# openxrlab/xrsfm

Measured on AMD Instinct MI355X. Metric: BA iterations/sec x (cams+points), higher is better.
Workload: dtype f64; 1 GPU; synthetic BAL-style L: 1000 cams / 500000 points / 2000000 obs, GBA accurate (ba_solver.cc:626-629), seed 4; parallelism=single GPU, linear_solver=cholesky (explicit reduced camera matrix, exact)

## Files before the change

### include/xrsfm_ba.h

```cpp
#ifndef XRSFM_BA_H
#define XRSFM_BA_H

#include <stddef.h>
#include <stdint.h>

#ifdef __cplusplus
extern "C" {
#endif

#define XRSFM_BA_VERSION 1

#define XRSFM_BA_OK 0
#define XRSFM_BA_EINVAL (-1)
#define XRSFM_BA_ENODEV (-2)
#define XRSFM_BA_ENOMEM (-3)
#define XRSFM_BA_ECOMM (-4)
#define XRSFM_BA_ESTATE (-5)
#define XRSFM_BA_ETOOBIG (-6)
#define XRSFM_BA_EINTERNAL (-7)
#define XRSFM_BA_ESINGULAR (-8)

#define XRSFM_BA_SIMPLE_PINHOLE 0
#define XRSFM_BA_PINHOLE 1
#define XRSFM_BA_SIMPLE_RADIAL 2
// ... 302 lines not shown

int xrsfm_ba_debug_gram_schedule(int n_cams, int32_t *n_inst, int32_t *n_inst_all, uint16_t *entries);

int xrsfm_ba_debug_chol_plan(const xrsfm_ba_problem *problem, int32_t stats[8], int32_t *cam_offset, int32_t *facts);

int xrsfm_ba_debug_device_pack_check(const xrsfm_ba_problem *problem, int32_t *field, int32_t *index);

int xrsfm_ba_debug_set_block_pattern(xrsfm_ba_context *ctx, int n_pairs, const int32_t *row_col);

int xrsfm_ba_debug_cholesky_solve(xrsfm_ba_context *ctx, double radius, double *y, double *S_dense);

int xrsfm_ba_debug_reduced_system(xrsfm_ba_context *ctx, double radius, int32_t facts[16], int32_t *n_blocks, int32_t *blk_rc,
                                  double *blk, double *diag, double *b, double *y);

int xrsfm_ba_debug_wide(xrsfm_ba_context *ctx, double huber_a, double radius, double *cost, double *r, double *Jc, double *Jp,
                        double *Hcc_diag, double *gc, double *y);

int xrsfm_ba_debug_backsub(xrsfm_ba_context *ctx, double *part_model, double *part_step2, double *cand_points,
                           double *point_step, double *cand_cam_q, double *cand_cam_t);

int xrsfm_ba_debug_backsub_layout(xrsfm_ba_context *ctx, int32_t *pt_orig, int32_t *item_tiles, double *campart, int32_t flags[2],
                                  double *cand_intr, double *scale_c, double *scale_p);

int xrsfm_ba_debug_stored_j(xrsfm_ba_context *ctx, int32_t *stored);

int xrsfm_ba_debug_lin_scalars(xrsfm_ba_context *ctx, double out[4]);

#ifdef __cplusplus
}
#endif
#endif
```

### xrsfm_amd/capi.py

```python
from __future__ import annotations

import ctypes as C
import os

import numpy as np

from . import _build

_c_double_p = C.POINTER(C.c_double)
_c_int32_p = C.POINTER(C.c_int32)
_c_uint8_p = C.POINTER(C.c_uint8)


class CProblem(C.Structure):
    _fields_ = [
        ("n_cams", C.c_int32), ("n_points", C.c_int32), ("n_obs", C.c_int32), ("n_intr", C.c_int32),
        ("cam_q", _c_double_p), ("cam_t", _c_double_p), ("cam_const", _c_uint8_p), ("cam_intr", _c_int32_p),
        ("intr_model", _c_int32_p), ("intr_params", _c_double_p),
        ("points", _c_double_p), ("point_const", _c_uint8_p),
        ("obs_cam", _c_int32_p), ("obs_pt", _c_int32_p), ("obs_uv", _c_double_p),
    ]


class CPgProblem(C.Structure):
# ... 71 lines not shown
        ("total_time_s", C.c_double), ("dom_kernel_ms", C.c_double),
        ("dom_kernel_launches", C.c_int32), ("dom_kernel_id", C.c_int32),
        ("linear_solver_used", C.c_int32), ("reserved", C.c_int32),
    ]

    def as_dict(self):
        return {f: getattr(self, f) for f, _ in self._fields_}


EXPORTS = [
    "xrsfm_ba_default_options", "xrsfm_ba_version", "xrsfm_ba_create", "xrsfm_ba_comm_unique_id",
    "xrsfm_ba_comm_init", "xrsfm_ba_run", "xrsfm_ba_reset", "xrsfm_ba_download", "xrsfm_ba_destroy",
    "xrsfm_ba_solve", "xrsfm_ba_filter_tracks", "xrsfm_ba_profile_entry", "xrsfm_ba_debug_linearize", "xrsfm_ba_debug_schur_product",
    "xrsfm_ba_debug_cholesky_solve", "xrsfm_ba_debug_set_block_pattern", "xrsfm_ba_debug_pack", "xrsfm_ba_debug_chol_plan", "xrsfm_ba_refine_pose", "xrsfm_ba_refine_pose_options", "xrsfm_ba_debug_comm_hook", "xrsfm_pg_default_options", "xrsfm_pg_solve", "xrsfm_ba_debug_pack_gram", "xrsfm_ba_debug_gram_schedule",
    "xrsfm_tag_default_options", "xrsfm_tag_refine", "xrsfm_ba_refine_poses", "xrsfm_ba_quiesce", "xrsfm_ba_debug_backsub", "xrsfm_ba_device_memory", "xrsfm_ba_download_intrinsics", "xrsfm_ba_debug_wide",
    "xrsfm_ba_debug_device_pack_check", "xrsfm_ba_warmup", "xrsfm_ba_debug_stored_j", "xrsfm_ba_debug_sgroup",
    "xrsfm_ba_debug_reduced_system", "xrsfm_ba_covariance", "xrsfm_ba_point_covariance", "xrsfm_ba_joint_covariance",
    "xrsfm_ba_map_covariance", "xrsfm_ba_debug_backsub_layout", "xrsfm_ba_run_batch", "xrsfm_ba_solve_batch",
    "xrsfm_ba_triangulate_options", "xrsfm_ba_triangulate_tracks", "xrsfm_ba_debug_lin_scalars",
    "xrsfm_ba_absolute_pose_options", "xrsfm_ba_absolute_pose", "xrsfm_ba_debug_pose_samples",
    "xrsfm_ba_two_view_options_default", "xrsfm_ba_two_view_init", "xrsfm_ba_debug_two_view_samples",
    "xrsfm_ba_verify_pairs_options", "xrsfm_ba_verify_pairs", "xrsfm_ba_debug_fund_samples",
    "xrsfm_ba_match_options_default", "xrsfm_ba_match_descriptors", "xrsfm_ba_debug_match_table",
]
EXPORTS_WITH_DIGITS = ["xrsfm_ba_debug_match_top2"]

CHOL_FACTS = ("T", "levels", "ordering", "schedule", "macro_levels", "split_levels", "la_depth", "fill_rest", "rest_apart", "packed",
              "bwd", "height_mask", "cw", "blocks", "n", "tiles_nz")
SCHEDULES = ("level", "panel", "lookahead")
BWD_FORMS = ("fused", "per_level", "all", "chunk", "push")


def _facts(v) -> dict:
    f = dict(zip(CHOL_FACTS, (int(x) for x in v)))
    f["schedule"] = SCHEDULES[f["schedule"]]
    f["bwd"] = BWD_FORMS[f["bwd"]]
    f["rest_apart"] = bool(f["rest_apart"]); f["packed"] = bool(f["packed"])
    f["heights"] = sorted(m * f["cw"] for m in range(1, 31) if (f["height_mask"] >> m) & 1)
    return f

SOLVER_PCG, SOLVER_CHOLESKY, SOLVER_AUTO = 0, 1, 2
SOLVER_RESIDENT = 3
BATCH_MAX = 4096
TRI_MAX_OBS = 128
TRI_LOCAL_BIT = 1 << 30
POSE_MAX_CORR = 8192
# ... 36 lines not shown
    lib.xrsfm_ba_run.argtypes = [vp, C.POINTER(COptions), C.POINTER(CSummary)]; lib.xrsfm_ba_run.restype = C.c_int
    lib.xrsfm_ba_reset.argtypes = [vp]; lib.xrsfm_ba_reset.restype = C.c_int
    lib.xrsfm_ba_download.argtypes = [vp, _c_double_p, _c_double_p, _c_double_p]; lib.xrsfm_ba_download.restype = C.c_int
    lib.xrsfm_ba_destroy.argtypes = [vp]; lib.xrsfm_ba_destroy.restype = None
    lib.xrsfm_ba_solve.argtypes = [C.POINTER(COptions), C.POINTER(CProblem), C.POINTER(CSummary)]; lib.xrsfm_ba_solve.restype = C.c_int
    lib.xrsfm_ba_filter_tracks.argtypes = [C.POINTER(CProblem), C.c_double, C.c_double, _c_uint8_p, _c_uint8_p, _c_double_p,
                                            _c_double_p, _c_int32_p]
    lib.xrsfm_ba_filter_tracks.restype = C.c_int
    lib.xrsfm_ba_debug_linearize.argtypes = [vp, C.c_double, C.c_int] + [_c_double_p] * 8
    lib.xrsfm_ba_debug_linearize.restype = C.c_int
    lib.xrsfm_ba_debug_schur_product.argtypes = [vp, C.c_double, _c_double_p, _c_double_p, _c_double_p]
    lib.xrsfm_ba_debug_schur_product.restype = C.c_int
    lib.xrsfm_ba_debug_cholesky_solve.argtypes = [vp, C.c_double, _c_double_p, _c_double_p]
    lib.xrsfm_ba_debug_cholesky_solve.restype = C.c_int
    if hasattr(lib, "xrsfm_ba_debug_stored_j"):
        lib.xrsfm_ba_debug_stored_j.argtypes = [vp, C.POINTER(C.c_int32)]
        lib.xrsfm_ba_debug_stored_j.restype = C.c_int
    if hasattr(lib, "xrsfm_ba_debug_backsub"):
        lib.xrsfm_ba_debug_backsub.argtypes = [vp] + [_c_double_p] * 6
        lib.xrsfm_ba_debug_backsub.restype = C.c_int
    if hasattr(lib, "xrsfm_ba_debug_backsub_layout"):
        lib.xrsfm_ba_debug_backsub_layout.argtypes = [vp, _c_int32_p, _c_int32_p, _c_double_p, _c_int32_p] + [_c_double_p] * 3
        lib.xrsfm_ba_debug_backsub_layout.restype = C.c_int
    lib.xrsfm_ba_debug_set_block_pattern.argtypes = [vp, C.c_int, _c_int32_p]
    lib.xrsfm_ba_debug_set_block_pattern.restype = C.c_int
    lib.xrsfm_pg_default_options.argtypes = [C.POINTER(CPgOptions)]
    lib.xrsfm_pg_default_options.restype = None
    lib.xrsfm_ba_refine_poses.argtypes = [C.POINTER(COptions), C.c_int32, _c_int32_p, _c_double_p, _c_int32_p, _c_double_p, _c_double_p,
                                          _c_uint8_p, _c_double_p, _c_double_p, C.POINTER(CSummary)]
    lib.xrsfm_ba_refine_poses.restype = C.c_int
    lib.xrsfm_pg_solve.argtypes = [C.POINTER(CPgOptions), C.POINTER(CPgProblem), C.POINTER(CPgSummary)]
    lib.xrsfm_pg_solve.restype = C.c_int
    lib.xrsfm_tag_default_options.argtypes = [C.POINTER(CPgOptions)]
    lib.xrsfm_tag_default_options.restype = None
    lib.xrsfm_tag_refine.argtypes = [C.POINTER(CPgOptions), C.POINTER(CTagProblem), C.c_int32, C.POINTER(CPgSummary)]
    lib.xrsfm_tag_refine.restype = C.c_int
    lib.xrsfm_ba_debug_comm_hook.argtypes = [C.c_void_p, C.c_int, C.c_int, ALLREDUCE_FN, C.c_void_p]
    lib.xrsfm_ba_debug_comm_hook.restype = C.c_int
    lib.xrsfm_ba_refine_pose_options.argtypes = [C.POINTER(COptions)]
    lib.xrsfm_ba_refine_pose_options.restype = None
    lib.xrsfm_ba_refine_pose.argtypes = [C.POINTER(COptions), C.c_int32, _c_double_p, C.c_int32, _c_double_p, _c_double_p, _c_uint8_p,
                                         _c_double_p, _c_double_p, C.POINTER(CSummary)]
    lib.xrsfm_ba_refine_pose.restype = C.c_int
    lib.xrsfm_ba_debug_pack_gram.argtypes = [C.POINTER(CProblem), _c_int32_p, _c_int32_p, _c_uint8_p, _c_int32_p]
    lib.xrsfm_ba_debug_pack_gram.restype = C.c_int
    lib.xrsfm_ba_debug_sgroup.argtypes = [C.POINTER(CProblem), C.c_int] + [_c_int32_p] * 7
# ... 304 lines not shown
        p = self.problem
        out = dict(r=np.zeros((p.n_obs, 2)), Jc=np.zeros((p.n_obs, 2, 9)), Jp=np.zeros((p.n_obs, 2, 3)), Hcc_diag=np.zeros((p.n_cams, 9)),
                   gc=np.zeros((p.n_cams, 9)))
        y = np.zeros((p.n_cams, 9)) if radius is not None else None
        cost = C.c_double(0)
        self.lib.xrsfm_ba_debug_wide.argtypes = [C.c_void_p, C.c_double, C.c_double, C.POINTER(C.c_double)] + [_c_double_p] * 6
        self.lib.xrsfm_ba_debug_wide.restype = C.c_int
        check(self.lib.xrsfm_ba_debug_wide(self._h, huber_a, float(radius or 1.0), C.byref(cost), _dp(out["r"]), _dp(out["Jc"]), _dp(out["Jp"]),
                                          _dp(out["Hcc_diag"]), _dp(out["gc"]), _dp(y)), "xrsfm_ba_debug_wide")
        out["cost"] = cost.value
        if y is not None:
            out["y"] = y
        return out

    def debug_backsub(self) -> dict:
        st = debug_pack(self.problem)
        ni, npk, nc = st["items"], st["active_points"], self.problem.n_cams
        out = dict(part_model=np.zeros(ni), part_step2=np.zeros(ni), cand_points=np.zeros((npk, 3)), point_step=np.zeros((npk, 3)),
                   cand_cam_q=np.zeros((nc, 4)), cand_cam_t=np.zeros((nc, 3)))
        check(self.lib.xrsfm_ba_debug_backsub(self._h, *[_dp(out[k]) for k in ("part_model", "part_step2", "cand_points", "point_step",
                                                                                  "cand_cam_q", "cand_cam_t")]), "debug_backsub")
        return out

    def debug_backsub_layout(self, after_backsub: bool = False, scales: bool = False) -> dict:
        st = debug_pack(self.problem)
        nc = self.problem.n_cams
        out = dict(pt_orig=np.zeros(st["active_points"], np.int32), item_tiles=np.zeros((st["items"], 2), np.int32))
        flags = np.zeros(2, np.int32)
        if after_backsub:
            out["campart"] = np.zeros((2, nc)); out["cand_intr"] = np.zeros((nc, 3))
        if scales:
            cw = 9 if (self.problem.cam_const & 4).any() else 6
            out["scale_c"] = np.zeros((nc, cw)); out["scale_p"] = np.zeros((st["active_points"], 3))
        i32 = lambda a: a.ctypes.data_as(_c_int32_p)
        check(self.lib.xrsfm_ba_debug_backsub_layout(self._h, i32(out["pt_orig"]), i32(out["item_tiles"]), _dp(out.get("campart")), i32(flags),
                                                     _dp(out.get("cand_intr")), _dp(out.get("scale_c")), _dp(out.get("scale_p"))),
              "debug_backsub_layout")
        out["step_prep"] = bool(flags[0]); out["stored_j"] = bool(flags[1])
        out["slot_obs"] = st["slot_obs"]
        return out

    def debug_backsub_caller_order(self) -> dict:
        raw = self.debug_backsub()
        lay = self.debug_backsub_layout(after_backsub=True, scales=True)
        p = self.problem
        po = lay["pt_orig"]
# ... 552 lines not shown
```

### xrsfm_amd/csrc/ba_chol.h

```cpp
#pragma once
#include "ba_kernels.h"
#include "ba_pack.h"

namespace xba {

constexpr int kNB = 64;
constexpr int kLdT = 66;
constexpr int kCamsPerTileDev = 10;

struct CholDev {
    int n, n_pad, T;
    double* S;
    const int* tmap; size_t ld; size_t tstride;
    double* Linv;
    double* y;
    double* rhs;
    double* x;
    const int* cam_off;
    const int* tile_rows;
    int cw, cpt;
};

__device__ __forceinline__ double* tile_ptr(const CholDev& c, int i, int k) {
    return c.tmap ? c.S + (size_t)c.tmap[i * c.T + k] * c.tstride : c.S + (size_t)(i * kNB) * c.ld + k * kNB;
// ... 294 lines not shown
    double* const smem = smem_all + (size_t)wave * wld;
    XBA_STAMP(0, 0);
    SGroup sg{0, 1, smem, wld, 0.0, 0.0, -1};
    if (MERGED && sgrp) {
        const int code = __builtin_amdgcn_readfirstlane(sgrp[pos]);
        sg.idx = code & 15; sg.len = code >> 4;
    }
    const int entry = item_list[MERGED ? n_list - 1 - pos : pos];
    Item it;
    if (GRAM) { it.first_tile = entry; it.n_tiles = 1; }
    else it = d.items[entry];
    if (GRAM || it.n_tiles == 1) {
        int dt0 = -1, dt1 = -1;
        int g4_se = 0, g4_n = 0;
        if (GRAM) {
            const int C0 = d.tile_ncam[it.first_tile];
            const int* src = pair_dst + n_obs_pairs + d.tile_gt_off[it.first_tile];
            const int a0 = lane / kGramTabLd, b0 = lane - kGramTabLd * a0;
            const int a1 = (lane + kWave) / kGramTabLd, b1 = lane + kWave - kGramTabLd * a1;
            if (b0 > a0 && b0 < C0) dt0 = src[a0 * C0 + b0];
            if (b1 > a1 && b1 < C0 && a1 < kGramTabLd) dt1 = src[a1 * C0 + b1];
            if (NIK <= 2 && gram4) g4_se = gram4_sched_load<6>(C0, lane, g4_n);
        }
        const SlotCtx s = load_slot(d, it.first_tile, lane);
        const int cp = d.slot_campos_s[s.slot];
        const int cidx_raw = GRAM ? (int)d.slot_cidx[s.slot] : 0;
        const int L = d.tile_stride[it.first_tile];
        int g_pos = kWave - 1, g_pk0 = 0, g_pk1 = 0, g_pk2 = 0;
        if (GRAM && L == 0) {
            const int C0 = d.tile_ncam[it.first_tile];
            const int* trun = d.tile_run + (size_t)it.first_tile * kTileRunLd;
            const int c0 = lane / 14, c1 = (lane + 64) / 14, c2 = (lane + 128) / 14;
            g_pos = (int)d.slot_gpos[s.slot];
            if (c0 < C0) g_pk0 = trun[c0];
            if (c1 < C0) g_pk1 = trun[c1];
            if (c2 < C0) g_pk2 = trun[c2];
        }
        double V[18];
        int npair = 0, pbase = 0;
        {
            double o28[28];
            XBA_STAMP(0, 1);
            if (s.valid) {
                double hcv[6], gv[3];
                {
                    const double* hc = (PREP ? d.Hpp : d.Hc) + 6 * (size_t)s.pt;
                    const double* g = d.gp + 3 * (size_t)s.pt;
#pragma unroll
                    for (int k = 0; k < 6; ++k) hcv[k] = hc[k];
                    gv[0] = g[0]; gv[1] = g[1]; gv[2] = g[2];
                }
                double F[12], E[6], r0, r1;
                load_FE_rc(d, s.slot, s.cam, s.pt, F, E, r0, r1);
                if (PREP) { double hf[6]; point_factor(hcv, radius, hf);
#pragma unroll
                    for (int k = 0; k < 6; ++k) hcv[k] = hf[k]; }
                XBA_STAMP(0, 2);
                pairs_V<PREP>(F, E, hcv, V);
                XBA_STAMP(0, 3);
                pairs_diag<PREP>(F, V, hcv, gv, o28);
            } else if (PREP) { dead_values(V); dead_values(o28); }
            else {
#pragma unroll
                for (int k = 0; k < 18; ++k) V[k] = XBA_DEAD;
#pragma unroll
                for (int k = 0; k < 28; ++k) o28[k] = XBA_DEAD;
// ... 1407 lines not shown
```

### xrsfm_amd/csrc/ba_kernels.h

```cpp
#pragma once
#include "ba_math.h"

namespace xba {

constexpr int kWave = 64;
constexpr int kBlock = 256;
constexpr int kWavesPerBlock = kBlock / kWave;

struct Item { int first_tile; int n_tiles; };

struct PcgStatus {
    double rz;
    double rr;
    double bb;
    double pq;
    int it;
    int done;
    unsigned arrived;
};

enum Scal {
    S_COST = 0, S_XNORM2_PTS, S_MODEL, S_STEP2_PTS, S_COST_CAND, S_STEP2_CAMS, S_XNORM2_CAMS,
    S_GRADMAX_PTS, S_GRADMAX_CAMS,
    S_BWD_ERR,
    S_COUNT = 16
};

struct __attribute__((aligned(16))) CamLin {
    double M[9];
    double sq[3];
    double st[3];
    double pad;
};
static_assert(sizeof(CamLin) == 128, "CamLin must be 128 bytes");

struct Dev {
    int n_cams, n_pts, n_tiles, n_slots, n_items;
    const int* slot_cam; const int* slot_pt; const int* slot_campos;
    const double* slot_u; const double* slot_v;
    const Item* items;
    const int* tile_stride;
    const int* tile_maxlen;
    const int* tile_ncam;
    const int* tile_gt_off;
    const unsigned char* slot_cidx;
    const int* slot_campos_g;
    const unsigned char* slot_gpos;
    const int* tile_run;
    const int* cam_ptr_g;
    const int* slot_campos_s; const int* cam_ptr_s;
    CamRec* cam; CamRec* cam_cand; const int* cam_model; const unsigned char* cam_const; const int* cam_ptr;
    double* cam_act;
    double* P; double* P_cand; const unsigned char* pt_const;
    double* scale_c; double* scale_p;
    double* rt; double* Jp;
    double huber_a;
    CamLin* camrec;
    double* Hpp; double* gp; double* Hinv;
    double* Hc;
    double* camlin;
// ... 178 lines not shown
__global__ __launch_bounds__(256) void k_sgroup_remap_ptr(const int* __restrict__ src, int n, const int* __restrict__ pos, int* __restrict__ dst) {
    const int i = blockIdx.x * 256 + threadIdx.x;
    if (i < n) dst[i] = pos[src[i]];
}

struct SlotCtx {
    int slot, cam, pt, lane;
    bool valid, head;
};

__device__ __forceinline__ SlotCtx load_slot(const Dev& d, int tile, int lane) {
    SlotCtx s;
    s.lane = lane;
    s.slot = tile * kWave + lane;
    s.cam = d.slot_cam[s.slot];
    s.pt = d.slot_pt[s.slot];
    s.valid = s.cam >= 0;
    const int prev = __shfl_up(s.pt, 1, kWave);
    s.head = s.valid && (lane == 0 || prev != s.pt);
    return s;
}


__device__ __forceinline__ void robust_obs(const double (&M)[9], const double t[3], const double* intr, int model, const double Pw[3],
                                           double u, double v, double huber_a, Proj& pr, double& rho, double& sw) {
    project<true>(M, t, intr, model, Pw, u, v, pr);
    double rho1;
    rho = huber(pr.r0 * pr.r0 + pr.r1 * pr.r1, huber_a, rho1);
    sw = sqrt(rho1);
}

__device__ __forceinline__ void obs_rj(const Dev& d, int slot, int cam, const double (&M)[9], const double Pw[3],
                                       double& r0, double& r1, double (&j)[6]) {
    const CamRec& c = d.cam[cam];
    const double t[3] = {c.t[0], c.t[1], c.t[2]};
    Proj pr;
    double rho, sw;
    robust_obs(M, t, c.intr, d.cam_model[cam], Pw, d.slot_u[slot], d.slot_v[slot], d.huber_a, pr, rho, sw);
    r0 = pr.r0 * sw; r1 = pr.r1 * sw;
#pragma unroll
    for (int k = 0; k < 6; ++k) j[k] = pr.jp[k] * sw;
    asm("" : "+v"(r0), "+v"(r1));
#pragma unroll
    for (int k = 0; k < 6; ++k) asm("" : "+v"(j[k]));
}

__device__ __forceinline__ void fe_from_j(const Dev& d, const CamLin& c, const double (&M)[9], int pt, const double P0, const double P1,
                                          const double P2, const double (&j)[6], double (&F)[12], double (&E)[6]) {
    const double rp0 = M[0] * P0 + M[1] * P1 + M[2] * P2;
    const double rp1 = M[3] * P0 + M[4] * P1 + M[5] * P2;
    const double rp2 = M[6] * P0 + M[7] * P1 + M[8] * P2;
    const double* spp = d.scale_p + 3 * (size_t)pt;
    const double mp = d.pt_const[pt] ? 0.0 : 1.0;
    const double sp0 = spp[0] * mp, sp1 = spp[1] * mp, sp2 = spp[2] * mp;
#pragma unroll
    for (int row = 0; row < 2; ++row) {
        const double a = j[3 * row], b = j[3 * row + 1], cc = j[3 * row + 2];
        F[6 * row + 0] = -2.0 * (b * rp2 - cc * rp1) * c.sq[0];
        F[6 * row + 1] = -2.0 * (cc * rp0 - a * rp2) * c.sq[1];
        F[6 * row + 2] = -2.0 * (a * rp1 - b * rp0) * c.sq[2];
        F[6 * row + 3] = a * c.st[0];
        F[6 * row + 4] = b * c.st[1];
        F[6 * row + 5] = cc * c.st[2];
        E[3 * row + 0] = (a * M[0] + b * M[3] + cc * M[6]) * sp0;
        E[3 * row + 1] = (a * M[1] + b * M[4] + cc * M[7]) * sp1;
        E[3 * row + 2] = (a * M[2] + b * M[5] + cc * M[8]) * sp2;
    }
}

__device__ __forceinline__ void load_FE(const Dev& d, int slot, int cam, int pt, double (&F)[12], double (&E)[6]) {
    const size_t ns = (size_t)d.n_slots;
    double j[6];
#pragma unroll
    for (int k = 0; k < 6; ++k) j[k] = d.Jp[k * ns + slot];
    const CamLin& c = d.camrec[cam];
    double M[9];
#pragma unroll
    for (int k = 0; k < 9; ++k) M[k] = c.M[k];
    const double* P = d.P + 3 * (size_t)pt;
    fe_from_j(d, c, M, pt, P[0], P[1], P[2], j, F, E);
}

__device__ __forceinline__ void load_FE_rc(const Dev& d, int slot, int cam, int pt, double (&F)[12], double (&E)[6], double& r0, double& r1) {
    const size_t ns = (size_t)d.n_slots;
    const CamLin& c = d.camrec[cam];
    double M[9];
#pragma unroll
    for (int k = 0; k < 9; ++k) M[k] = c.M[k];
    const double* P = d.P + 3 * (size_t)pt;
    const double Pw[3] = {P[0], P[1], P[2]};
    double j[6];
    if (d.Jp) {
#pragma unroll
        for (int k = 0; k < 6; ++k) j[k] = d.Jp[k * ns + slot];
        r0 = d.rt[slot]; r1 = d.rt[ns + slot];
    } else {
        obs_rj(d, slot, cam, M, Pw, r0, r1, j);
    }
    fe_from_j(d, c, M, pt, Pw[0], Pw[1], Pw[2], j, F, E);
}

__device__ __forceinline__ void cam_lin_one(const Dev& d, int c, const double q[4], CamLin* __restrict__ out) {
    CamLin r;
    quat_to_mat(q, r.M);
    const unsigned cc = d.cam_const[c];
    const double* sc = d.scale_c + 6 * (size_t)c;
    for (int k = 0; k < 3; ++k) { r.sq[k] = (cc & 1u) ? 0.0 : sc[k]; r.st[k] = (cc & 2u) ? 0.0 : sc[3 + k]; }
    r.pad = 0.0;
    out[c] = r;
}
__global__ void k_cam_lin(Dev d) {
    const int c = blockIdx.x * blockDim.x + threadIdx.x;
    if (c >= d.n_cams) return;
    const double q[4] = {d.cam[c].q[0], d.cam[c].q[1], d.cam[c].q[2], d.cam[c].q[3]};
    cam_lin_one(d, c, q, d.camrec);
}

template <bool LONG>
__device__ __forceinline__ void linearize_item(const Dev& d, const Item& it, int item, int lane, double huber_a) {
    constexpr bool is_long = LONG;
    extern __shared__ __attribute__((aligned(16))) double lin_smem_acc[];
    double* acc = lin_smem_acc + (threadIdx.x >> 6) * (kWave * 13);
// ... 1120 lines not shown
            const int slot = (it.first_tile + tl) * kWave + lane;
            const int cam = d.slot_cam[slot];
            if (cam >= 0) {
                const double* y = d.px + 6 * (size_t)cam;
                double F[12], E[6], r0, r1;
                load_FE_rc(d, slot, cam, pt0, F, E, r0, r1);
                double v0 = 0.0, v1 = 0.0;
#pragma unroll
                for (int k = 0; k < 6; ++k) { v0 += F[k] * y[k]; v1 += F[6 + k] * y[k]; }
                const double m0 = v0 + E[0] * u[0] + E[1] * u[1] + E[2] * u[2];
                const double m1 = v1 + E[3] * u[0] + E[4] * u[1] + E[5] * u[2];
                model += m0 * (r0 - 0.5 * m0) + m1 * (r1 - 0.5 * m1);
            }
        }
    }
}

#if XBA_BACKSUB_WAVES > 0
#define XBA_BACKSUB_LEAN_WAVES XBA_BACKSUB_WAVES
#else
#define XBA_BACKSUB_LEAN_WAVES 5
#endif
constexpr int kBsLdsH = 16 * kWave, kBsLdsW = 4 * kWave;
constexpr int kBsLdsWave = 4 * kBsLdsH + 2 * kBsLdsW;

__device__ __forceinline__ double rounded(double x) { asm("" : "+v"(x)); return x; }

__device__ __forceinline__ void load_vE_rc(const Dev& d, int slot, int cam, const double (&Pw)[3], const double* __restrict__ sp, double mp,
                                           double (&spm)[3], double (&E)[6], double& v0, double& v1, double& r0, double& r1) {
    const size_t ns = (size_t)d.n_slots;
    const CamLin& c = d.camrec[cam];
    double M[9];
#pragma unroll
    for (int k = 0; k < 9; ++k) M[k] = c.M[k];
    double j[6];
    if (d.Jp) {
#pragma unroll
        for (int k = 0; k < 6; ++k) j[k] = d.Jp[k * ns + slot];
        r0 = d.rt[slot]; r1 = d.rt[ns + slot];
    } else {
        obs_rj(d, slot, cam, M, Pw, r0, r1, j);
    }
    const double rp0 = M[0] * Pw[0] + M[1] * Pw[1] + M[2] * Pw[2];
    const double rp1 = M[3] * Pw[0] + M[4] * Pw[1] + M[5] * Pw[2];
    const double rp2 = M[6] * Pw[0] + M[7] * Pw[1] + M[8] * Pw[2];
    const double* y = d.px + 6 * (size_t)cam;
#pragma unroll
    for (int k = 0; k < 3; ++k) spm[k] = sp[k] * mp;
    double v[2];
#pragma unroll
    for (int row = 0; row < 2; ++row) {
        const double a = j[3 * row], b = j[3 * row + 1], cc = j[3 * row + 2];
        double vr = 0.0;
        vr += -2.0 * (b * rp2 - cc * rp1) * c.sq[0] * y[0];
        vr += -2.0 * (cc * rp0 - a * rp2) * c.sq[1] * y[1];
        vr += -2.0 * (a * rp1 - b * rp0) * c.sq[2] * y[2];
        vr += a * c.st[0] * y[3];
        vr += b * c.st[1] * y[4];
        vr += cc * c.st[2] * y[5];
        v[row] = vr;
        E[3 * row + 0] = (a * M[0] + b * M[3] + cc * M[6]) * spm[0];
        E[3 * row + 1] = (a * M[1] + b * M[4] + cc * M[7]) * spm[1];
        E[3 * row + 2] = (a * M[2] + b * M[5] + cc * M[8]) * spm[2];
    }
    v0 = v[0]; v1 = v[1];
}

template <bool PREP, bool YP>
__global__ __launch_bounds__(kBlock) __attribute__((amdgpu_waves_per_eu(XBA_BACKSUB_LEAN_WAVES, XBA_BACKSUB_LEAN_WAVES)))
void k_backsub(Dev d, int n_item_blocks, CamLin* __restrict__ camrec_cand, double radius) {
    typedef __attribute__((address_space(1))) const void* gptr;
    typedef __attribute__((address_space(3))) void* lptr;
    __shared__ __attribute__((aligned(16))) unsigned char hg[kWavesPerBlock * kBsLdsWave];
    if ((int)blockIdx.x >= n_item_blocks) {
        const int c = (blockIdx.x - n_item_blocks) * kBlock + threadIdx.x;
        if (c < d.n_cams) cam_update_one(d, c, d.px + 6 * (size_t)c, camrec_cand);
        return;
    }
    const int lane = threadIdx.x & (kWave - 1);
    const int wave = __builtin_amdgcn_readfirstlane(threadIdx.x >> 6);
    const int item = blockIdx.x * kWavesPerBlock + wave;
    if (item >= d.n_items) return;
    const Item it = d.items[item];
    if (it.n_tiles != 1) return;
    const SlotCtx s = load_slot(d, it.first_tile, lane);
    const int maxlen = d.tile_maxlen[it.first_tile];
    unsigned char* const lw = hg + wave * kBsLdsWave;
    if (s.head) {
        const double* h = (PREP ? d.Hpp : d.Hinv) + 6 * (size_t)s.pt;
        const unsigned char* g = reinterpret_cast<const unsigned char*>(d.gp + 3 * (size_t)s.pt);
        __builtin_amdgcn_global_load_lds((gptr)h, (lptr)lw, 16, 0, 0);
        __builtin_amdgcn_global_load_lds((gptr)(h + 2), (lptr)(lw + kBsLdsH), 16, 0, 0);
        __builtin_amdgcn_global_load_lds((gptr)(h + 4), (lptr)(lw + 2 * kBsLdsH), 16, 0, 0);
        __builtin_amdgcn_global_load_lds((gptr)g, (lptr)(lw + 3 * kBsLdsH), 16, 0, 0);
        __builtin_amdgcn_global_load_lds((gptr)(g + 16), (lptr)(lw + 4 * kBsLdsH), 4, 0, 0);
        __builtin_amdgcn_global_load_lds((gptr)(g + 20), (lptr)(lw + 4 * kBsLdsH + kBsLdsW), 4, 0, 0);
    }
    double model = 0.0, step2 = 0.0;
    double E[6], v0, v1, r0, r1;
    double w[3] = {0, 0, 0};
    double spm[3], Pv[3];
    bool var = false;
    if (s.valid) {
        const double* P = d.P + 3 * (size_t)s.pt;
        var = !d.pt_const[s.pt];
        const double mp = var ? 1.0 : 0.0;
#pragma unroll
        for (int k = 0; k < 3; ++k) Pv[k] = P[k];
        load_vE_rc(d, s.slot, s.cam, Pv, d.scale_p + 3 * (size_t)s.pt, mp, spm, E, v0, v1, r0, r1);
#pragma unroll
        for (int k = 0; k < 3; ++k) w[k] = rounded(E[k] * v0) + E[3 + k] * v1;
    } else { dead_values(spm); dead_values(Pv); dead_values(E); XBA_DEAD_VALUE(v0); XBA_DEAD_VALUE(v1); XBA_DEAD_VALUE(r0); XBA_DEAD_VALUE(r1); }
    seg_reduce<3>(w, s.pt, lane, maxlen);
    double u[3];
    if (s.head) {
        asm volatile("s_waitcnt vmcnt(0)" ::: "memory");
        const double2* hq = reinterpret_cast<const double2*>(lw) + lane;
        const double2 h01 = hq[0], h23 = hq[kWave], h45 = hq[2 * kWave];
        const double hh[6] = {h01.x, h01.y, h23.x, h23.y, h45.x, h45.y};
        const unsigned* gq = reinterpret_cast<const unsigned*>(lw + 3 * kBsLdsH);
        const unsigned g0 = gq[4 * lane], g1 = gq[4 * lane + 1], g2 = gq[4 * lane + 2], g3 = gq[4 * lane + 3], g4 = gq[4 * kWave + lane], g5 = gq[5 * kWave + lane];
        const double a0 = __hiloint2double((int)g1, (int)g0) - w[0], a1 = __hiloint2double((int)g3, (int)g2) - w[1],
                     a2 = __hiloint2double((int)g5, (int)g4) - w[2];
        if (PREP) {
            double cf[6];
            point_factor(hh, radius, cf);
            const double s0 = cf[0] * a0, s1 = rounded(cf[1] * a0) + cf[3] * a1, s2 = cf[2] * a0 + rounded(cf[4] * a1) + cf[5] * a2;
            u[0] = cf[0] * s0 + rounded(cf[1] * s1) + cf[2] * s2;
            u[1] = cf[3] * s1 + rounded(cf[4] * s2);
            u[2] = cf[5] * s2;
        } else {
            u[0] = hh[0] * a0 + rounded(hh[1] * a1) + hh[2] * a2;
// ... 241 lines not shown
```

### xrsfm_amd/csrc/xrsfm_ba.hip

```cpp
#include <dlfcn.h>
#include <hip/hip_runtime.h>

#include <algorithm>
#include <chrono>
#include <condition_variable>
#include <deque>
#include <cmath>
#include <cstdio>
#include <cstdlib>
#include <cstring>
#include <map>
#include <mutex>
#include <thread>
#include <type_traits>
#include <vector>

#include "../../include/xrsfm_ba.h"
#include "ba_chol.h"
#include "ba_cov.h"
#include "ba_filter.h"
#include "ba_kernels.h"
#include "ba_lba.h"
#include "ba_pack.h"
#include "ba_plan.h"
// ... 2246 lines not shown
    if (c->wide) {
        TRY(dev_alloc(c, &c->w.Fw, ns * 18)); TRY(dev_alloc(c, &c->w.Ew, ns * 6));
        TRY(dev_alloc(c, &c->w.scale_c, nc * kW)); TRY(dev_alloc(c, &c->w.camlin, nc * 18));
        TRY(dev_alloc(c, &c->w.px, nc * kW + kNB));
        TRY(dev_alloc(c, &c->w.scat, (size_t)(k.n_obs > 0 ? k.n_obs : 1) * kWS));
        c->cam_intr_host.assign(p->cam_intr, p->cam_intr + p->n_cams);
    }
    TRY(dev_alloc(c, &c->part2, (size_t)kTailJobs * kTailGrid));
    TRY(dev_alloc(c, &c->ticket, (size_t)32 * 9));
    {
        unsigned char* gpos = nullptr; int* trun = nullptr;
        TRY(dev_alloc(c, &gpos, ns ? ns : 1)); TRY(dev_alloc(c, &trun, (size_t)std::max(1, k.n_tiles) * kTileRunLd));
        if (k.n_tiles > 0) hipLaunchKernelGGL(k_gram_runs, dim3(cdiv(k.n_tiles, 4)), dim3(256), 0, c->stream, d.slot_cam, d.slot_cidx, d.tile_ncam, k.n_tiles, gpos, trun);
        d.slot_gpos = gpos; d.tile_run = trun;
    }
#undef TRY
    {
        const char* fz = std::getenv("XRSFM_BA_FUSED");
        c->fused = !(fz && fz[0] == '0');
        const char* pf = std::getenv("XRSFM_BA_PREP_FUSED");
        c->prep_fused = !(pf && pf[0] == '0');
        const char* bl = std::getenv("XRSFM_BA_BACKSUB_LEAN");
        c->backsub_lean = !(bl && bl[0] == '0');
        const char* pc = std::getenv("XRSFM_BA_PCG_COARSE");
        c->pcg_coarse = !(pc && pc[0] == '0');
    }
    if (hipMemsetAsync(d.scal, 0, sizeof(double) * S_COUNT, c->stream) != hipSuccess || hipMemsetAsync(d.st, 0, sizeof(PcgStatus), c->stream) != hipSuccess ||
        hipMemsetAsync(c->ticket, 0, sizeof(unsigned) * 32 * 9, c->stream) != hipSuccess ||
        hipStreamSynchronize(c->stream) != hipSuccess) { xrsfm_ba_destroy(c); return XRSFM_BA_ENODEV; }
    timer.mark("work buffers");
    *out = c;
    return XRSFM_BA_OK;
}

int xrsfm_ba_comm_unique_id(unsigned char id[128]) {
    if (!id) return XRSFM_BA_EINVAL;
    if (!load_rccl()) return XRSFM_BA_ECOMM;
    UniqueId u;
    if (g_rccl.GetUniqueId(&u) != 0) return XRSFM_BA_ECOMM;
    memcpy(id, u.internal, 128);
    return 0;
}

int xrsfm_ba_comm_init(xrsfm_ba_context* c, int n_ranks, int rank, const unsigned char id[128]) {
    if (c && c->poisoned) return XRSFM_BA_ESTATE;
    if (!c || !id || n_ranks < 1 || n_ranks > kMaxRanks || rank < 0 || rank >= n_ranks) return XRSFM_BA_EINVAL;
// ... 2131 lines not shown
    if (item_tiles) for (size_t i = 0; i < k.items.size(); ++i) item_tiles[i] = k.items[i];
    if (flags) { flags[0] = (c->wide || c->step_prep) ? 1 : 0; flags[1] = (c->wide || d.Jp != nullptr) ? 1 : 0; }
    if (scale_c || scale_p) {
        if (!c->linearized) return XRSFM_BA_ESTATE;
        HIPCHK(hipSetDevice(c->device));
        HIPCHK(hipStreamSynchronize(c->stream));
        const size_t ncw = (size_t)d.n_cams * (c->wide ? kW : 6);
        if (scale_c && ncw) HIPCHK(hipMemcpy(scale_c, c->wide ? c->w.scale_c : d.scale_c, ncw * sizeof(double), hipMemcpyDeviceToHost));
        if (scale_p && d.n_pts) HIPCHK(hipMemcpy(scale_p, d.scale_p, 3 * (size_t)d.n_pts * sizeof(double), hipMemcpyDeviceToHost));
    }
    if (campart || cand_intr) {
        if (!c->step_valid || !c->backsub_done) return XRSFM_BA_ESTATE;
        HIPCHK(hipSetDevice(c->device));
        if (campart && d.n_cams) HIPCHK(hipMemcpy(campart, d.campart, 2 * (size_t)d.n_cams * sizeof(double), hipMemcpyDeviceToHost));
        if (cand_intr && d.n_cams) {
            std::vector<CamRec> cams(d.n_cams);
            HIPCHK(hipMemcpy(cams.data(), d.cam_cand, sizeof(CamRec) * (size_t)d.n_cams, hipMemcpyDeviceToHost));
            for (int i = 0; i < d.n_cams; ++i) for (int j = 0; j < 3; ++j) cand_intr[3 * (size_t)i + j] = cams[i].intr[j];
        }
    }
    return 0;
}

int xrsfm_ba_debug_device_pack_check(const xrsfm_ba_problem* p, int32_t* field, int32_t* index) {
    if (!p || !field || !index) return XRSFM_BA_EINVAL;
    *field = 0; *index = -1;
    return no_throw([&]() -> int {
        Packed h;
        int e = pack_problem(*p, h, problem_is_wide(p));
        if (e) return e;
        xrsfm_ba_context* c = nullptr;
        g_force_device_pack = 1;
        e = xrsfm_ba_create(p, 0, &c);
        g_force_device_pack = -1;
        if (e) return e;
        struct Guard { xrsfm_ba_context* c; ~Guard() { xrsfm_ba_destroy(c); } } guard{c};
        if (!c->dev_packed) { *field = -100; return 0; }
        if ((e = ensure_host_pack(c, 2))) return e;
        const Packed& k = c->pk;
        auto diff = [&](int f, long long i) { *field = f; *index = (int32_t)i; return 0; };
        if (k.n_cams != h.n_cams || k.n_pts != h.n_pts || k.n_obs != h.n_obs || k.n_tiles != h.n_tiles || k.n_slots != h.n_slots ||
            k.n_gt_cells != h.n_gt_cells || k.n_cam_entries != h.n_cam_entries || k.n_cam_entries_g != h.n_cam_entries_g ||
            k.n_var_q != h.n_var_q || k.n_var_t != h.n_var_t || k.n_var_p != h.n_var_p) return diff(1, 0);
        auto cmp = [&](int f, const auto& a, const auto& b) -> bool {
            if (a.size() != b.size()) { diff(f, -2); return false; }
            for (size_t i = 0; i < a.size(); ++i) if (a[i] != b[i]) { diff(f, (long long)i); return false; }
// ... 52 lines not shown
```

Measured before the change: 1.137 billion cam-pts*iter/s.

## Stage per-tile camera records into LDS for merged Schur and backsub kernels

For single-tile items with at most eight distinct cameras, the wave cooperatively loads the camera linearization, pose/intrinsics, model and (for backsub) camera step into shared memory with 16-byte vector loads. Each lane then reads its camera data from LDS instead of issuing scattered per-lane global gathers of the same few camera records. This aims to cut redundant global traffic and gather latency in the Schur pair-accumulation and back-substitution kernels. It costs extra LDS per wave in backsub, which may reduce occupancy, and it adds a wave barrier. It is on by default and can be disabled with an environment variable.

After: 1.243 billion cam-pts*iter/s, median of 6. 9.4% higher.

```diff
diff --git a/include/xrsfm_ba.h b/include/xrsfm_ba.h
--- a/include/xrsfm_ba.h
+++ b/include/xrsfm_ba.h
@@ -348,6 +348,8 @@
 int xrsfm_ba_debug_backsub_layout(xrsfm_ba_context *ctx, int32_t *pt_orig, int32_t *item_tiles, double *campart, int32_t flags[2],
                                   double *cand_intr, double *scale_c, double *scale_p);
 
+int xrsfm_ba_debug_cam_stage(xrsfm_ba_context *ctx, int32_t counts[2]);
+
 int xrsfm_ba_debug_stored_j(xrsfm_ba_context *ctx, int32_t *stored);
 
 int xrsfm_ba_debug_lin_scalars(xrsfm_ba_context *ctx, double out[4]);
diff --git a/xrsfm_amd/capi.py b/xrsfm_amd/capi.py
--- a/xrsfm_amd/capi.py
+++ b/xrsfm_amd/capi.py
@@ -117,6 +117,7 @@
     "xrsfm_ba_two_view_options_default", "xrsfm_ba_two_view_init", "xrsfm_ba_debug_two_view_samples",
     "xrsfm_ba_verify_pairs_options", "xrsfm_ba_verify_pairs", "xrsfm_ba_debug_fund_samples",
     "xrsfm_ba_match_options_default", "xrsfm_ba_match_descriptors", "xrsfm_ba_debug_match_table",
+    "xrsfm_ba_debug_cam_stage",
 ]
 EXPORTS_WITH_DIGITS = ["xrsfm_ba_debug_match_top2"]
 
@@ -199,6 +200,9 @@
     if hasattr(lib, "xrsfm_ba_debug_backsub_layout"):
         lib.xrsfm_ba_debug_backsub_layout.argtypes = [vp, _c_int32_p, _c_int32_p, _c_double_p, _c_int32_p] + [_c_double_p] * 3
         lib.xrsfm_ba_debug_backsub_layout.restype = C.c_int
+    if hasattr(lib, "xrsfm_ba_debug_cam_stage"):
+        lib.xrsfm_ba_debug_cam_stage.argtypes = [vp, _c_int32_p]
+        lib.xrsfm_ba_debug_cam_stage.restype = C.c_int
     lib.xrsfm_ba_debug_set_block_pattern.argtypes = [vp, C.c_int, _c_int32_p]
     lib.xrsfm_ba_debug_set_block_pattern.restype = C.c_int
     lib.xrsfm_pg_default_options.argtypes = [C.POINTER(CPgOptions)]
@@ -549,6 +553,11 @@
                                                                                   "cand_cam_q", "cand_cam_t")]), "debug_backsub")
         return out
 
+    def debug_cam_stage(self) -> tuple:
+        counts = np.zeros(2, np.int32)
+        check(self.lib.xrsfm_ba_debug_cam_stage(self._h, counts.ctypes.data_as(_c_int32_p)), "debug_cam_stage")
+        return int(counts[0]), int(counts[1])
+
     def debug_backsub_layout(self, after_backsub: bool = False, scales: bool = False) -> dict:
         st = debug_pack(self.problem)
         nc = self.problem.n_cams
diff --git a/xrsfm_amd/csrc/ba_chol.h b/xrsfm_amd/csrc/ba_chol.h
--- a/xrsfm_amd/csrc/ba_chol.h
+++ b/xrsfm_amd/csrc/ba_chol.h
@@ -340,6 +340,7 @@
             if (b1 > a1 && b1 < C0 && a1 < kGramTabLd) dt1 = src[a1 * C0 + b1];
             if (NIK <= 2 && gram4) g4_se = gram4_sched_load<6>(C0, lane, g4_n);
         }
+        const int run = (MERGED && d.cam_stage) ? d.tile_run[(size_t)it.first_tile * kTileRunLd + min(lane, kTileRunLd - 1)] : 0;
         const SlotCtx s = load_slot(d, it.first_tile, lane);
         const int cp = d.slot_campos_s[s.slot];
         const int cidx_raw = GRAM ? (int)d.slot_cidx[s.slot] : 0;
@@ -359,7 +360,37 @@
         {
             double o28[28];
             XBA_STAMP(0, 1);
-            if (s.valid) {
+            constexpr int kSpRecLd = 30;
+            const bool staged = MERGED && cam_staged(d.cam_stage, 1, d.tile_ncam[it.first_tile]);
+            if (staged) {
+                const int C0 = d.tile_ncam[it.first_tile];
+                const int camL = stage_tile_cam(C0, run, s.cam, lane);
+                const int model = d.cam_model[camL];
+                CamStage st;
+                st.request(C0, camL, lane, {d.camrec, 128u, 0u, 8}, {d.cam, 128u, 32u, 6});
+                st.deposit(smem, kSpRecLd);
+                *reinterpret_cast<int*>(smem + min(lane, C0 - 1) * kSpRecLd + 28) = model;
+                stage_done();
+            }
+            if (staged && s.valid) {
+                double hcv[6], gv[3];
+                {
+                    const double* hc = (PREP ? d.Hpp : d.Hc) + 6 * (size_t)s.pt;
+                    const double* g = d.gp + 3 * (size_t)s.pt;
+#pragma unroll
+                    for (int k = 0; k < 6; ++k) hcv[k] = hc[k];
+                    gv[0] = g[0]; gv[1] = g[1]; gv[2] = g[2];
+                }
+                double F[12], E[6], r0, r1;
+                const double* r = smem + cidx_raw * kSpRecLd;
+                const CamOps o = {r, r + 16, r + 20, nullptr, reinterpret_cast<const int*>(r + 28), d.slot_u + s.slot, d.slot_v + s.slot};
+                load_FE_at(d, s.slot, s.pt, o, d.P + 3 * (size_t)s.pt, F, E, r0, r1);
+                if (PREP) { double hf[6]; point_factor(hcv, radius, hf);
+#pragma unroll
+                    for (int k = 0; k < 6; ++k) hcv[k] = hf[k]; }
+                pairs_V<PREP>(F, E, hcv, V);
+                pairs_diag<PREP>(F, V, hcv, gv, o28);
+            } else if (s.valid) {
                 double hcv[6], gv[3];
                 {
                     const double* hc = (PREP ? d.Hpp : d.Hc) + 6 * (size_t)s.pt;
diff --git a/xrsfm_amd/csrc/ba_kernels.h b/xrsfm_amd/csrc/ba_kernels.h
--- a/xrsfm_amd/csrc/ba_kernels.h
+++ b/xrsfm_amd/csrc/ba_kernels.h
@@ -36,6 +36,7 @@
 
 struct Dev {
     int n_cams, n_pts, n_tiles, n_slots, n_items;
+    int cam_stage;
     const int* slot_cam; const int* slot_pt; const int* slot_campos;
     const double* slot_u; const double* slot_v;
     const Item* items;
@@ -260,6 +261,40 @@
 }
 
 
+constexpr int kCamStageMax = 8;
+__host__ __device__ inline bool cam_staged(int on, int n_tiles, int C) { return on && n_tiles == 1 && C > 0 && C <= kCamStageMax; }
+
+__device__ __forceinline__ int stage_tile_cam(int C, int run, int cam, int lane) {
+    return __shfl(cam, (__shfl(run, min(lane, C - 1), kWave) >> 16) & 63, kWave);
+}
+struct StagePart { const void* base; unsigned stride, first; int n; };
+struct CamStage {
+    static constexpr int kPass = kCamStageMax / 4;
+    int p, ci[kPass];
+    double2 x[kPass];
+    __device__ __forceinline__ void request(int C, int camL, int lane, const StagePart a, const StagePart b, const StagePart c = {nullptr, 0u, 0u, 0}) {
+        p = min(lane & 15, a.n + b.n + c.n - 1);
+        const unsigned char* base = static_cast<const unsigned char*>(a.base);
+        unsigned stride = a.stride, piece = a.first + 16u * p;
+        if (p >= a.n) { base = static_cast<const unsigned char*>(b.base); stride = b.stride; piece = b.first + 16u * (p - a.n); }
+        if (c.n > 0 && p >= a.n + b.n) { base = static_cast<const unsigned char*>(c.base); stride = c.stride; piece = c.first + 16u * (p - a.n - b.n); }
+#pragma unroll
+        for (int k = 0; k < kPass; ++k) {
+            ci[k] = min(4 * k + (lane >> 4), C - 1);
+            x[k] = *reinterpret_cast<const double2*>(base + (__umul24((unsigned)__shfl(camL, ci[k], kWave), stride) + piece));
+        }
+    }
+    __device__ __forceinline__ void deposit(double* rec, int ld) const {
+#pragma unroll
+        for (int k = 0; k < kPass; ++k) *reinterpret_cast<double2*>(rec + ci[k] * ld + 2 * p) = x[k];
+    }
+};
+__device__ __forceinline__ void stage_done() {
+    __builtin_amdgcn_s_waitcnt(0xc07f);
+    __builtin_amdgcn_wave_barrier();
+}
+
+
 __device__ __forceinline__ void robust_obs(const double (&M)[9], const double t[3], const double* intr, int model, const double Pw[3],
                                            double u, double v, double huber_a, Proj& pr, double& rho, double& sw) {
     project<true>(M, t, intr, model, Pw, u, v, pr);
@@ -268,19 +303,23 @@
     sw = sqrt(rho1);
 }
 
+__device__ __forceinline__ void obs_rj_at(const double* tp, const double* intr, const int* model, const double* u, const double* v, double huber_a,
+                                          const double (&M)[9], const double Pw[3], double& r0, double& r1, double (&j)[6]) {
+    const double t[3] = {tp[0], tp[1], tp[2]};
+    Proj pr;
+    double rho, sw;
+    robust_obs(M, t, intr, *model, Pw, *u, *v, huber_a, pr, rho, sw);
+    r0 = pr.r0 * sw; r1 = pr.r1 * sw;
+#pragma unroll
+    for (int k = 0; k < 6; ++k) j[k] = pr.jp[k] * sw;
+    asm("" : "+v"(r0), "+v"(r1));
+#pragma unroll
+    for (int k = 0; k < 6; ++k) asm("" : "+v"(j[k]));
+}
 __device__ __forceinline__ void obs_rj(const Dev& d, int slot, int cam, const double (&M)[9], const double Pw[3],
                                        double& r0, double& r1, double (&j)[6]) {
     const CamRec& c = d.cam[cam];
-    const double t[3] = {c.t[0], c.t[1], c.t[2]};
-    Proj pr;
-    double rho, sw;
-    robust_obs(M, t, c.intr, d.cam_model[cam], Pw, d.slot_u[slot], d.slot_v[slot], d.huber_a, pr, rho, sw);
-    r0 = pr.r0 * sw; r1 = pr.r1 * sw;
-#pragma unroll
-    for (int k = 0; k < 6; ++k) j[k] = pr.jp[k] * sw;
-    asm("" : "+v"(r0), "+v"(r1));
-#pragma unroll
-    for (int k = 0; k < 6; ++k) asm("" : "+v"(j[k]));
+    obs_rj_at(c.t, c.intr, d.cam_model + cam, d.slot_u + slot, d.slot_v + slot, d.huber_a, M, Pw, r0, r1, j);
 }
 
 __device__ __forceinline__ void fe_from_j(const Dev& d, const CamLin& c, const double (&M)[9], int pt, const double P0, const double P1,
@@ -319,13 +358,22 @@
     fe_from_j(d, c, M, pt, P[0], P[1], P[2], j, F, E);
 }
 
-__device__ __forceinline__ void load_FE_rc(const Dev& d, int slot, int cam, int pt, double (&F)[12], double (&E)[6], double& r0, double& r1) {
+struct CamOps {
+    const double* lin;
+    const double* t;
+    const double* intr;
+    const double* y;
+    const int* model;
+    const double* u; const double* v;
+};
+
+__device__ __forceinline__ void load_FE_at(const Dev& d, int slot, int pt, const CamOps& o, const double* P, double (&F)[12], double (&E)[6],
+                                           double& r0, double& r1) {
     const size_t ns = (size_t)d.n_slots;
-    const CamLin& c = d.camrec[cam];
+    const CamLin& c = *reinterpret_cast<const CamLin*>(o.lin);
     double M[9];
 #pragma unroll
     for (int k = 0; k < 9; ++k) M[k] = c.M[k];
-    const double* P = d.P + 3 * (size_t)pt;
     const double Pw[3] = {P[0], P[1], P[2]};
     double j[6];
     if (d.Jp) {
@@ -333,9 +381,14 @@
         for (int k = 0; k < 6; ++k) j[k] = d.Jp[k * ns + slot];
         r0 = d.rt[slot]; r1 = d.rt[ns + slot];
     } else {
-        obs_rj(d, slot, cam, M, Pw, r0, r1, j);
+        obs_rj_at(o.t, o.intr, o.model, o.u, o.v, d.huber_a, M, Pw, r0, r1, j);
     }
     fe_from_j(d, c, M, pt, Pw[0], Pw[1], Pw[2], j, F, E);
+}
+__device__ __forceinline__ void load_FE_rc(const Dev& d, int slot, int cam, int pt, double (&F)[12], double (&E)[6], double& r0, double& r1) {
+    const CamRec& c = d.cam[cam];
+    const CamOps o = {reinterpret_cast<const double*>(d.camrec + cam), c.t, c.intr, nullptr, d.cam_model + cam, d.slot_u + slot, d.slot_v + slot};
+    load_FE_at(d, slot, pt, o, d.P + 3 * (size_t)pt, F, E, r0, r1);
 }
 
 __device__ __forceinline__ void cam_lin_one(const Dev& d, int c, const double q[4], CamLin* __restrict__ out) {
@@ -1502,29 +1555,30 @@
 #define XBA_BACKSUB_LEAN_WAVES 5
 #endif
 constexpr int kBsLdsH = 16 * kWave, kBsLdsW = 4 * kWave;
-constexpr int kBsLdsWave = 4 * kBsLdsH + 2 * kBsLdsW;
 
 __device__ __forceinline__ double rounded(double x) { asm("" : "+v"(x)); return x; }
 
-__device__ __forceinline__ void load_vE_rc(const Dev& d, int slot, int cam, const double (&Pw)[3], const double* __restrict__ sp, double mp,
+__device__ __forceinline__ void load_vE_rc(const Dev& d, int slot, const CamOps& c, const double (&Pw)[3],
+                                           const double* __restrict__ sp, double mp,
                                            double (&spm)[3], double (&E)[6], double& v0, double& v1, double& r0, double& r1) {
     const size_t ns = (size_t)d.n_slots;
-    const CamLin& c = d.camrec[cam];
+    const double* sq = c.lin + 9;
+    const double* st = c.lin + 12;
     double M[9];
 #pragma unroll
-    for (int k = 0; k < 9; ++k) M[k] = c.M[k];
+    for (int k = 0; k < 9; ++k) M[k] = c.lin[k];
     double j[6];
     if (d.Jp) {
 #pragma unroll
         for (int k = 0; k < 6; ++k) j[k] = d.Jp[k * ns + slot];
         r0 = d.rt[slot]; r1 = d.rt[ns + slot];
     } else {
-        obs_rj(d, slot, cam, M, Pw, r0, r1, j);
+        obs_rj_at(c.t, c.intr, c.model, c.u, c.v, d.huber_a, M, Pw, r0, r1, j);
     }
     const double rp0 = M[0] * Pw[0] + M[1] * Pw[1] + M[2] * Pw[2];
     const double rp1 = M[3] * Pw[0] + M[4] * Pw[1] + M[5] * Pw[2];
     const double rp2 = M[6] * Pw[0] + M[7] * Pw[1] + M[8] * Pw[2];
-    const double* y = d.px + 6 * (size_t)cam;
+    const double* y = c.y;
 #pragma unroll
     for (int k = 0; k < 3; ++k) spm[k] = sp[k] * mp;
     double v[2];
@@ -1532,18 +1586,34 @@
     for (int row = 0; row < 2; ++row) {
         const double a = j[3 * row], b = j[3 * row + 1], cc = j[3 * row + 2];
         double vr = 0.0;
-        vr += -2.0 * (b * rp2 - cc * rp1) * c.sq[0] * y[0];
-        vr += -2.0 * (cc * rp0 - a * rp2) * c.sq[1] * y[1];
-        vr += -2.0 * (a * rp1 - b * rp0) * c.sq[2] * y[2];
-        vr += a * c.st[0] * y[3];
-        vr += b * c.st[1] * y[4];
-        vr += cc * c.st[2] * y[5];
+        vr += -2.0 * (b * rp2 - cc * rp1) * sq[0] * y[0];
+        vr += -2.0 * (cc * rp0 - a * rp2) * sq[1] * y[1];
+        vr += -2.0 * (a * rp1 - b * rp0) * sq[2] * y[2];
+        vr += a * st[0] * y[3];
+        vr += b * st[1] * y[4];
+        vr += cc * st[2] * y[5];
         v[row] = vr;
         E[3 * row + 0] = (a * M[0] + b * M[3] + cc * M[6]) * spm[0];
         E[3 * row + 1] = (a * M[1] + b * M[4] + cc * M[7]) * spm[1];
         E[3 * row + 2] = (a * M[2] + b * M[5] + cc * M[8]) * spm[2];
     }
     v0 = v[0]; v1 = v[1];
+}
+
+constexpr int kBsRecLd = 36;
+constexpr int kBsLdsHead = 4 * kBsLdsH + 2 * kBsLdsW;
+constexpr int kBsLdsWave = kBsLdsHead + kCamStageMax * kBsRecLd * 8;
+__device__ __forceinline__ void backsub_stage_cams(const Dev& d, int C, int run, int cam, int lane, double* rec) {
+    const int cl = min(lane, C - 1);
+    const int camL = stage_tile_cam(C, run, cam, lane);
+    const double2 y45 = *reinterpret_cast<const double2*>(d.px + 6 * (size_t)camL + 4);
+    const int model = d.cam_model[camL];
+    CamStage st;
+    st.request(C, camL, lane, {d.camrec, 128u, 0u, 8}, {d.cam, 128u, 32u, 6}, {d.px, 48u, 0u, 2});
+    st.deposit(rec, kBsRecLd);
+    *reinterpret_cast<double2*>(rec + cl * kBsRecLd + 32) = y45;
+    *reinterpret_cast<int*>(rec + cl * kBsRecLd + 34) = model;
+    stage_done();
 }
 
 template <bool PREP, bool YP>
@@ -1563,6 +1633,7 @@
     if (item >= d.n_items) return;
     const Item it = d.items[item];
     if (it.n_tiles != 1) return;
+    const int run = d.cam_stage ? d.tile_run[(size_t)it.first_tile * kTileRunLd + min(lane, kTileRunLd - 1)] : 0;
     const SlotCtx s = load_slot(d, it.first_tile, lane);
     const int maxlen = d.tile_maxlen[it.first_tile];
     unsigned char* const lw = hg + wave * kBsLdsWave;
@@ -1581,13 +1652,39 @@
     double w[3] = {0, 0, 0};
     double spm[3], Pv[3];
     bool var = false;
-    if (s.valid) {
+    const int C = d.tile_ncam[it.first_tile];
+    if (cam_staged(d.cam_stage, 1, C)) {
+        double* const rec = reinterpret_cast<double*>(lw + kBsLdsHead);
+        double uo, vo;
+        int cidx = 0, fixed = 0;
+        if (s.valid) {
+            const double* P = d.P + 3 * (size_t)s.pt;
+            fixed = d.pt_const[s.pt];
+            cidx = d.slot_cidx[s.slot];
+            uo = d.slot_u[s.slot]; vo = d.slot_v[s.slot];
+#pragma unroll
+            for (int k = 0; k < 3; ++k) Pv[k] = P[k];
+        } else { dead_values(Pv); XBA_DEAD_VALUE(uo); XBA_DEAD_VALUE(vo); }
+        backsub_stage_cams(d, C, run, s.cam, lane, rec);
+        asm volatile("" : "+v"(cidx), "+v"(fixed));
+        var = s.valid && !fixed;
+        if (s.valid) {
+            const double* r = rec + cidx * kBsRecLd;
+            const CamOps ops = {r, r + 16, r + 20, r + 28, reinterpret_cast<const int*>(r + 34), &uo, &vo};
+            load_vE_rc(d, s.slot, ops, Pv, d.scale_p + 3 * (size_t)s.pt, var ? 1.0 : 0.0, spm, E, v0, v1, r0, r1);
+#pragma unroll
+            for (int k = 0; k < 3; ++k) w[k] = rounded(E[k] * v0) + E[3 + k] * v1;
+        } else { dead_values(spm); dead_values(E); XBA_DEAD_VALUE(v0); XBA_DEAD_VALUE(v1); XBA_DEAD_VALUE(r0); XBA_DEAD_VALUE(r1); }
+    } else if (s.valid) {
         const double* P = d.P + 3 * (size_t)s.pt;
         var = !d.pt_const[s.pt];
         const double mp = var ? 1.0 : 0.0;
 #pragma unroll
         for (int k = 0; k < 3; ++k) Pv[k] = P[k];
-        load_vE_rc(d, s.slot, s.cam, Pv, d.scale_p + 3 * (size_t)s.pt, mp, spm, E, v0, v1, r0, r1);
+        const CamRec& cr = d.cam[s.cam];
+        const CamOps ops = {reinterpret_cast<const double*>(d.camrec + s.cam), cr.t, cr.intr, d.px + 6 * (size_t)s.cam, d.cam_model + s.cam,
+                            d.slot_u + s.slot, d.slot_v + s.slot};
+        load_vE_rc(d, s.slot, ops, Pv, d.scale_p + 3 * (size_t)s.pt, mp, spm, E, v0, v1, r0, r1);
 #pragma unroll
         for (int k = 0; k < 3; ++k) w[k] = rounded(E[k] * v0) + E[3 + k] * v1;
     } else { dead_values(spm); dead_values(Pv); dead_values(E); XBA_DEAD_VALUE(v0); XBA_DEAD_VALUE(v1); XBA_DEAD_VALUE(r0); XBA_DEAD_VALUE(r1); }
diff --git a/xrsfm_amd/csrc/xrsfm_ba.hip b/xrsfm_amd/csrc/xrsfm_ba.hip
--- a/xrsfm_amd/csrc/xrsfm_ba.hip
+++ b/xrsfm_amd/csrc/xrsfm_ba.hip
@@ -2292,6 +2292,8 @@
         c->prep_fused = !(pf && pf[0] == '0');
         const char* bl = std::getenv("XRSFM_BA_BACKSUB_LEAN");
         c->backsub_lean = !(bl && bl[0] == '0');
+        const char* cs = std::getenv("XRSFM_BA_CAM_STAGE");
+        d.cam_stage = !(cs && cs[0] == '0') && d.n_cams < (1 << 24);
         const char* pc = std::getenv("XRSFM_BA_PCG_COARSE");
         c->pcg_coarse = !(pc && pc[0] == '0');
     }
@@ -4469,6 +4471,23 @@
     return 0;
 }
 
+int xrsfm_ba_debug_cam_stage(xrsfm_ba_context* c, int32_t counts[2]) {
+    if (c && c->poisoned) return XRSFM_BA_ESTATE;
+    if (!c || !counts) return XRSFM_BA_EINVAL;
+    counts[0] = counts[1] = 0;
+    if (c->wide) return 0;
+    return no_throw([&]() -> int {
+        if (int e = ensure_host_pack(c, 1)) return e;
+        const Packed& k = c->pk;
+        for (size_t i = 0; i + 1 < k.items.size(); i += 2) {
+            const int first = k.items[i], n = k.items[i + 1];
+            if (cam_staged(c->d.cam_stage, n, k.tile_ncam[first])) counts[0] += 1;
+            else counts[1] += n;
+        }
+        return 0;
+    });
+}
+
 int xrsfm_ba_debug_device_pack_check(const xrsfm_ba_problem* p, int32_t* field, int32_t* index) {
     if (!p || !field || !index) return XRSFM_BA_EINVAL;
     *field = 0; *index = -1;
```
